# shravan-d/SculptMate

Measured on AMD Instinct MI355X. Metric: meshes/sec + ms/image, TripoSR 256^3 grid, at 1/2/4/8 MI355X, higher is better.
Workload: dtype fp32-equivalent (bf16 3-limb split, 24 bits, fp32 accumulate) density MLP / f32 tables, SiLU, marching cubes / bf16 transformer [filtered grid: an fp16 one-product pass decides the SIGN away from the level, every value marching cubes reads carries the three-limb value: mesh bit-identical to the full

## Files before the change

include/sculpt_hip.h:

```cpp
#ifndef SCULPT_HIP_H
#define SCULPT_HIP_H

#include <stddef.h>
#include <stdint.h>

#ifdef __cplusplus
extern "C" {
#endif

#define SCULPT_ABI_VERSION 4

typedef void *sculpt_stream_t;

int sculpt_version(void);
const char *sculpt_source_digest(void);
const char *sculpt_last_error(void);
int sculpt_device_count(void);
int sculpt_stream_create_cu_mask(int first_cu, int n_cus, sculpt_stream_t *stream_out);
int sculpt_stream_destroy(sculpt_stream_t stream);

size_t sculpt_mlp_packed_bytes(int in_channels, int n_hidden_64);
int sculpt_mlp_pack(const float *const *W_host, const float *const *b_host, int n_layers,
                    const int *dims_host, void *packed_host, size_t packed_bytes);

int sculpt_triplane_query(const float *planes, int C, int H, int W, const void *mlp_packed,
                          int n_hidden_64, const float *points, int64_t N, float radius, float density_bias,
                          float *density, float *features, float *density_act, float *color,
                          sculpt_stream_t stream);

#define SCULPT_QUERY_ALIGN_CORNERS 1u
#define SCULPT_QUERY_CHANNEL_LAST 2u
int sculpt_planes_channel_last(const float *planes , int C, int H, int W, float *out ,
                               sculpt_stream_t stream);
int sculpt_triplane_query_ex(const float *planes, int C, int H, int W, const void *mlp_packed,
                             int n_hidden_64, const float *points, int64_t N, float radius, float density_bias,
                             unsigned flags, float *density, float *features, float *density_act, float *color,
                             sculpt_stream_t stream);

int sculpt_render_rays(const float *planes_cl , int C, int H, int W,
                       const void *mlp_packed, int n_hidden_64,
                       const float *rays_o, const float *rays_d , int64_t n_rays,
                       float radius, float density_bias,
                       const float *t_vals , int S,
                       float *comp_rgb ,
                       float *opacity ,
                       float *z_vals  ,
                       float *weights ,
                       sculpt_stream_t stream);

int sculpt_render_passes(const float *planes_cl , int C, int H, int W,
                         const void *mlp_packed, int n_hidden_64,
                         const float *rays_o, const float *rays_d , int64_t n_rays,
                         float radius, float density_bias,
                         const float *t_vals , int S,
                         float *comp_rgb ,
                         float *opacity ,
                         float *z_vals  ,
                         float *weights ,
                         float *depth_sum  ,
                         float *normal_sum ,
                         float *premul     ,
                         sculpt_stream_t stream);

int sculpt_bake_scene_color(const float *planes_cl , int C, int H, int W,
                            const void *mlp_packed, int n_hidden_64,
                            const float *v_pos , size_t nv,
                            const void *faces , int faces_i64, size_t nf,
                            const float *rast , int res,
                            float radius,
                            float *color , uint8_t *mask ,
                            sculpt_stream_t stream);

int sculpt_corner_tangents(const float *v_pos , size_t nv, const void *faces , int faces_i64, size_t nf,
                           const float *uvs , const float *corner_normals ,
                           float *tangents , sculpt_stream_t stream);

int sculpt_bake_scene_normal(const float *planes_cl , int C, int H, int W,
                             const void *mlp_packed, int n_hidden_64,
                             const float *v_pos , size_t nv,
                             const void *faces , int faces_i64, size_t nf,
                             const float *rast , int res,
                             float radius,
                             const float *corner_normals , const float *corner_tangents ,
                             float *normal , uint8_t *mask ,
                             sculpt_stream_t stream);

int sculpt_triplane_density_grad(const float *planes_cl , int C, int H, int W,
                                 const void *mlp_packed, int n_hidden_64,
                                 const float *points , long long N, float radius, int flags ,
                                 float *grad , float *normal , float *density ,
                                 sculpt_stream_t stream);

size_t sculpt_density_grid_workspace_bytes(int R, int nx);
int sculpt_plane_features(const float *planes, int C, int H, int W, const void *mlp_packed,
                          const float *axis_coords, int R, int x_begin, int x_end, float radius,
                          void *workspace, sculpt_stream_t stream);
int sculpt_plane_features_ex(const float *planes, int C, int H, int W, const void *mlp_packed,
                             const float *axis_coords, int R, int x_begin, int x_end, float radius, unsigned flags,
                             void *workspace, sculpt_stream_t stream);
int sculpt_density_grid(const void *mlp_packed, int n_hidden_64, int R, int x_begin, int x_end,
                        float density_bias, float out_add, const void *workspace, float *out,
                        sculpt_stream_t stream);
#define SCULPT_DENSITY_BF16L3 4u
int sculpt_density_grid_ex(const void *mlp_packed, int n_hidden_64, int R, int x_begin, int x_end,
                           float density_bias, float out_add, const void *workspace, float *out, unsigned flags,
                           sculpt_stream_t stream);
#define SCULPT_FILTER_STATS_WORDS 12
#define SCULPT_FILTER_COARSE_FP16 8u
#define SCULPT_FILTER_MARK_ALL 16u
#define SCULPT_FILTER_PASS_A 32u
#define SCULPT_FILTER_PASS_B 64u
#define SCULPT_FILTER_PASS_C 128u
size_t sculpt_density_filter_workspace_bytes(int R, int nx);
int sculpt_density_grid_filtered(const void *mlp_packed, int n_hidden_64, int R, int x_begin, int x_end, float density_bias,
                                 float out_add, float margin, const void *workspace, void *filter_workspace, float *out,
                                 unsigned flags, sculpt_stream_t stream);
size_t sculpt_density_filter_sign_offset(int R, int nx);
int sculpt_density_filter_stats(const void *filter_workspace, int32_t *stats , sculpt_stream_t stream);
int sculpt_grid_decode(const void *mlp_packed, int n_hidden_64, int R, int x_begin, int x_end, float density_bias,
                       float out_add, const void *workspace, float *density_act, float *features, sculpt_stream_t stream);

#define SCULPT_MC_FACES_I64 1u
#define SCULPT_MC_REFERENCE_ORDER 2u
#define SCULPT_MC_USE_CLASSIC 4u
#define SCULPT_MC_SLAB 8u
#define SCULPT_MC_SLAB_HALO_LOW 16u
#define SCULPT_MC_SIGNED 32u
#define SCULPT_ERR_MC_LEVEL 11
#define SCULPT_ERR_MC_EMPTY 12
#define SCULPT_ERR_MC_NAN 13
#define SCULPT_ERR_MC_WORKSPACE 14
#define SCULPT_ERR_MC_NO_COUNT 15

size_t sculpt_mc_workspace_bytes(int n0, int n1, int n2);
size_t sculpt_mc_workspace_bytes_for(int n0, int n1, int n2, int64_t max_active_cells);
int sculpt_mc_count(const float *vol, int n0, int n1, int n2, double level, unsigned flags,
                    void *workspace, int64_t *n_verts_host, int64_t *n_faces_host,
                    float *minmax_host , sculpt_stream_t stream);
int sculpt_mc_emit(const float *vol, int n0, int n1, int n2, double level, unsigned flags,
                   void *workspace, float vert_div, float vert_mul, float vert_add,
                   int axis0_offset ,
                   float *verts, void *faces, int *top_plane_map , sculpt_stream_t stream);
int sculpt_mc_count_launch(const float *vol, int n0, int n1, int n2, double level, unsigned flags, void *workspace,
                           sculpt_stream_t stream);
int sculpt_mc_count_launch_signed(const float *vol, const uint32_t *sign_planes, int words_per_row, int n0, int n1, int n2,
                                  double level, unsigned flags, void *workspace, sculpt_stream_t stream);
int sculpt_mc_count_read(int n0, int n1, int n2, double level, unsigned flags, const void *workspace, int64_t *n_verts_host,
                         int64_t *n_faces_host, float *minmax_host , sculpt_stream_t stream);
int sculpt_mc_count_launch_for(const float *vol, const uint32_t *sign_planes , int words_per_row, int n0, int n1, int n2,
                               double level, unsigned flags, int64_t max_active_cells, void *workspace, sculpt_stream_t stream);
int sculpt_mc_count_read_ex(int n0, int n1, int n2, double level, unsigned flags, const void *workspace, int64_t *n_verts_host,
                            int64_t *n_faces_host, float *minmax_host , int64_t *n_active_host ,
                            sculpt_stream_t stream);
int sculpt_mc_emit_capped(const float *vol, int n0, int n1, int n2, double level, unsigned flags, void *workspace, float vert_div,
                          float vert_mul, float vert_add, int axis0_offset, float *verts, int64_t cap_verts, void *faces,
                          int64_t cap_faces, int *top_plane_map , sculpt_stream_t stream);

#define SCULPT_SN_INDEX_I64 1u
#define SCULPT_ERR_SN_EMPTY 17
size_t sculpt_surface_nets_workspace_bytes(int n0, int n1, int n2);
int sculpt_surface_nets_count(const float *vol, const uint32_t *sign_planes , int words_per_row, int n0, int n1, int n2,
                              double level, unsigned flags, void *workspace, int64_t *n_verts_host, int64_t *n_quads_host,
                              sculpt_stream_t stream);
int sculpt_surface_nets_emit(const float *vol, int n0, int n1, int n2, double level, unsigned flags, void *workspace, float vert_div,
                             float vert_mul, float vert_add, float *verts, void *quads , void *faces ,
                             sculpt_stream_t stream);

#define SCULPT_CC_KEEP_NONE 0
#define SCULPT_CC_KEEP_LARGEST 1
#define SCULPT_CC_KEEP_MIN_FACES 2
#define SCULPT_CC_KEEP_FRACTION 3
#define SCULPT_ERR_MESH_COMPONENTS 16
size_t sculpt_mesh_components_workspace_bytes(int64_t n_vertices, int64_t n_faces);
int sculpt_mesh_components_launch(const void *faces, int faces_i64, int64_t n_faces, int64_t n_vertices, int rule, int64_t min_faces,
                                  double fraction, void *workspace, sculpt_stream_t stream);
int sculpt_mesh_components_read(const void *workspace, int64_t *counts_host );
int sculpt_mesh_components_compact(const float *vertices, const void *faces, int faces_i64, int64_t n_faces, int64_t n_vertices,
                                   void *workspace, float *out_vertices, int64_t cap_vertices, void *out_faces, int64_t cap_faces,
                                   int64_t *vertex_index, int64_t *face_index, sculpt_stream_t stream);
// ... 387 lines not shown
```

sculptmate_amd/_lib.py:

```python
import ctypes
import os

import torch

_HERE = os.path.dirname(os.path.abspath(__file__))
SO_PATH = os.path.join(_HERE, "libsculpt_hip.so")


class SculptError(RuntimeError):
    def __init__(self, msg, code=1):
        super().__init__(msg)
        self.code = code


if not os.path.exists(SO_PATH):
    raise ImportError(
        "sculptmate_amd: %s is missing -- build it with `python -m sculptmate_amd.build` "
        "(or __graft_entry__.build()); there is no CPU fallback." % SO_PATH)


def _load_matching_library():
    from . import build as _build

    if os.environ.get("SCULPT_ALLOW_STALE_LIB") == "1":
# ... 202 lines not shown
    "sculpt_catmull_classify": (_i, [_vp, _vp, _vp, _vp, _vp]),
    "sculpt_catmull_refine": (_i, [_vp, _vp, _vp, _vp, _vp, _i, _vp, _vp, _vp, _vp, _vp]),
    "sculpt_surface_closest": (_i, [_vp, _i64, _vp, _vp, _vp, _i64, _vp, _vp, _vp, _vp, _d, _vp, _vp, _vp, _vp]),
    "sculpt_surface_cells": (_i, [_vp, _i64, _vp, _vp, _vp]),
    "sculpt_surface_pack": (_i, [_vp, _vp, _i64, _vp, _vp]),
    "sculpt_surface_weights": (_i, [_vp, _vp, _i64, _vp, _vp, _vp, _vp]),
    "sculpt_surface_sample": (_i, [_vp, _vp, _i64, _vp, _i64, ctypes.c_uint64, _vp, _vp, _vp, _vp]),
    "sculpt_surface_winding": (_i, [_vp, _i64, _vp, _vp, _vp, _i64, _vp, _vp, _vp, _vp, _vp, _vp]),
    "sculpt_surface_winding_lattice": (_i, [_vp, _d, _i, _i, _i, _vp, _vp, _i64, _vp, _vp, _vp, _vp, _vp, _vp, _vp]),
    "sculpt_lattice_active_blocks": (_i64, [_i, _i, _i]),
    "sculpt_lattice_active_corners": (_i, [_vp, _i, _i, _i, _vp, _vp, _i64, _vp]),
    "sculpt_sdf_fill": (_i, [_vp, _vp, _i, _i, _i, _vp, _vp, _i64, _d, _vp]),
    "sculpt_surface_ray_cast": (_i, [_vp, _vp, _i64, _vp, _vp, _vp, _i64, _vp, _vp, _vp, _vp, _d, _d, _d, _vp, _vp, _vp, _vp]),
    "sculpt_surface_occlusion": (_i, [_vp, _vp, _i64, _vp, _vp, _i, _f, _f, _vp, _vp, _i64, _vp, _vp, _vp, _vp, _d, _vp, _vp]),
    "sculpt_bake_occlusion": (_i, [_vp, _i, _vp, _sz, _vp, _i, _sz, _vp, _vp, _i, _f, _f, _f, _vp, _vp, _i64, _vp, _vp, _vp, _vp, _d, _vp,
                                   _vp, _vp]),
    "sculpt_surface_render": (_i, [_vp, _vp, _i64, _i64, _i64, _vp, _vp, _i64, _vp, _vp, _vp, _vp, _d, _vp, _f, _vp, _d, _vp, _vp]),
    "sculpt_triplane_project": (_i, [_vp, _i, _i, _i, _vp, _i, _vp, ctypes.c_longlong, _f, _i, _f, _i, _f, _f, _vp, _vp, _vp, _vp, _vp]),
    "sculpt_mesh_unfold": (_i, [_vp, _vp, _vp, _i64, _i64, _i, _vp, _vp, _vp]),
    "sculpt_bake_scene_surface": (_i, [_vp, _i, _i, _i, _vp, _i, _vp, _sz, _vp, _i, _sz, _vp, _i, _f, _vp, _vp, _f, _i, _f, _f, _vp, _vp,
                                       _vp, _vp, _vp, _vp, _vp]),
    "sculpt_bake_texel_list_workspace_bytes": (_sz, [_i]),
    "sculpt_bake_texel_list": (_i, [_vp, _sz, _vp, _i, _sz, _vp, _vp, _i, _vp, _vp, _vp, _vp, _vp, _vp, _vp, _vp, _vp, _vp, _vp]),
    "sculpt_triplane_project_along": (_i, [_vp, _i, _i, _i, _vp, _i, _vp, _vp, ctypes.c_longlong, _vp, _f, _i, _f, _i, _f, _f, _vp,
                                           ctypes.c_longlong, _vp, _vp, _vp, _vp, _vp]),
    "rasterize_cpu": (None, [_vp, _sz, _vp, _sz, ctypes.c_longlong, _vp]),
    "interpolate_cpu": (None, [_vp, _sz, _vp, _sz, _vp, ctypes.c_longlong, _vp]),
}

for _name, (_res, _args) in SIGNATURES.items():
    _fn = getattr(lib, _name)
    _fn.restype = _res
    _fn.argtypes = _args

def rmd_undo_bytes(nv):
    return ((nv + 3) & ~3) + 4


class RmdTopo(ctypes.Structure):
    _fields_ = [("F", _vp), ("skeys", _vp), ("she", _vp), ("es", _vp), ("fe", _vp), ("vfs", _vp), ("vfc", _vp), ("bnd", _vp),
                ("nf", _i64), ("nv", _i64), ("ne", _i64)]


class CatmullTopo(ctypes.Structure):
    _fields_ = [("F", _vp), ("skeys", _vp), ("she", _vp), ("es", _vp), ("fe", _vp), ("vfs", _vp), ("vfc", _vp),
                ("nf", _i64), ("nv", _i64), ("ne", _i64), ("k", ctypes.c_int32)]


class RenderMaterial(ctypes.Structure):
    _fields_ = [("uvs", _vp), ("texture", _vp), ("normal_map", _vp), ("corner_normals", _vp), ("corner_tangents", _vp),
                ("occlusion_map", _vp), ("vertex_colors", _vp), ("vertex_normals", _vp), ("vertex_occlusion", _vp),
                ("texture_res", _i), ("normal_map_res", _i), ("occlusion_map_res", _i), ("vertex_color_channels", _i)]


class RenderOutputs(ctypes.Structure):
    _fields_ = [("color", _vp), ("shaded", _vp), ("opacity", _vp), ("rgba", _vp), ("depth", _vp), ("normal", _vp), ("occlusion", _vp),
                ("face", _vp)]


class LnFold(ctypes.Structure):
    _fields_ = [("stats_in", _vp), ("slots_in", _i), ("colsum", _vp), ("eps", _f), ("stats_out", _vp), ("stats_ld", _i),
                ("rows_per_image", _i)]


MC_FACES_I64 = 1
MC_REFERENCE_ORDER = 2
MC_USE_CLASSIC = 4
MC_SLAB = 8
MC_SLAB_HALO_LOW = 16
MC_SIGNED = 32
LIMBS_BF16X3, LIMBS_F16X2 = 0, 1
ERR_MC_LEVEL = 11
ERR_MC_EMPTY = 12
ERR_MC_NAN = 13
ERR_MC_WORKSPACE = 14
ERR_MC_NO_COUNT = 15
ERR_MESH_COMPONENTS = 16
SN_INDEX_I64 = 1
ERR_SN_EMPTY = 17
CC_KEEP_NONE, CC_KEEP_LARGEST, CC_KEEP_MIN_FACES, CC_KEEP_FRACTION = 0, 1, 2, 3
EPI_NONE, EPI_GELU, EPI_GEGLU, EPI_RELU = 0, 1, 2, 3
QUERY_ALIGN_CORNERS = 1
QUERY_CHANNEL_LAST = 2
DENSITY_BF16L3 = 4
FILTER_COARSE_FP16 = 8
FILTER_MARK_ALL = 16
FILTER_PASS_A, FILTER_PASS_B, FILTER_PASS_C = 32, 64, 128
F32_EXACT, F32_BF16L3 = 0, 1


def last_error():
    return (lib.sculpt_last_error() or b"").decode("utf-8", "replace")


def check(rc):
    if rc != 0:
        raise SculptError(last_error() or ("sculpt error %d" % rc), rc)


def form_has(var, token):
    return any(t == token or t.startswith(token + "=") for t in os.environ.get(var, "").split(",") if t)
```

sculptmate_amd/csrc/triplane.hip:

```cpp
#include <math.h>
#include <stdlib.h>
#include <string.h>

#include <vector>

#include "common.h"
#include "triplane_mlp.h"

namespace sculpt {

static inline uint16_t host_f32_to_bf16(float f) {
    uint32_t u;
    memcpy(&u, &f, 4);
    if ((u & 0x7fffffffu) > 0x7f800000u) return (uint16_t)((u >> 16) | 0x40);
    return (uint16_t)((u + 0x7fffu + ((u >> 16) & 1u)) >> 16);
}
static inline float host_bf16_to_f32(uint16_t v) {
    uint32_t u = (uint32_t)v << 16;
    float f;
    memcpy(&f, &u, 4);
    return f;
}

static void pack_layout(int K0, int NH, MlpPackHeader *hd) {
// ... 85 lines not shown
            if (features) { features[3 * n] = f0; features[3 * n + 1] = f1; features[3 * n + 2] = f2; }
            if (color) {
                color[3 * n] = color_f(f0);
                color[3 * n + 1] = color_f(f1);
                color[3 * n + 2] = color_f(f2);
            }
        }
    }
}

template <int C, bool AC = false>
__global__ __launch_bounds__(256) void plane_features_kernel(
    const float *__restrict__ planes, int H, int W, const float *__restrict__ blob,
    const float *__restrict__ axis, int R, int x_begin, int nx, float radius, float span,
    float *__restrict__ FA, float *__restrict__ FB, float *__restrict__ FC) {
    __shared__ __attribute__((aligned(16))) float wl[C][64];
    __shared__ __attribute__((aligned(16))) float bl[64];
    const MlpPackHeader hd = *reinterpret_cast<const MlpPackHeader *>(blob);
    const int K0 = hd.K0;
    const int lane = threadIdx.x & 63, w = threadIdx.x >> 6;
    const int bgroups = (R + 3) / 4;
    const long perA = (long)((nx + 63) / 64) * bgroups, perC = (long)((R + 63) / 64) * bgroups;
    int k, na;
    long rest;
    float *dst;
    {
        const long blk = blockIdx.x;
        if (blk < perA) { k = 0; rest = blk; na = nx; dst = FA; }
        else if (blk < 2 * perA) { k = 1; rest = blk - perA; na = nx; dst = FB; }
        else { k = 2; rest = blk - 2 * perA; na = R; dst = FC; }
    }
    (void)perC;
    const int a = (int)(rest / bgroups) * 64 + lane;
    const int b = (int)(rest % bgroups) * 4 + w;
    for (int i = threadIdx.x; i < C * 64; i += 256) {
        const int c = i >> 6, jj = i & 63;
        const int hh = jj >> 5, tt = (jj >> 4) & 1, rr = jj & 15;
        wl[c][jj] = blob[hd.off_w0raw + (long)nrow(tt, rr, hh) * K0 + k * C + c];
    }
    if (threadIdx.x < 64) {
        const int jj = threadIdx.x, hh = jj >> 5, tt = (jj >> 4) & 1, rr = jj & 15;
        bl[jj] = (k == 0) ? blob[hd.off_b0raw + nrow(tt, rr, hh)] : 0.f;
    }
    __syncthreads();
    if (b >= R) return;
    const bool live = a < na;
    const int ac = live ? a : na - 1;
    const int ia = (k == 2) ? ac : ac + x_begin;
    const float gx = to_unit(axis[ia], radius, span), gy = to_unit(axis[b], radius, span);
    Tap1 tx = tap_of<AC>(gx, W), ty = tap_of<AC>(gy, H);
    const float wx = tx.w1, ex = 1.0f - wx, wy = ty.w1, ey = 1.0f - wy;
    const int x0 = tx.i0, x1 = x0 + 1, y0 = ty.i0, y1 = y0 + 1;
    const bool vx0 = x0 >= 0 && x0 < W, vx1 = x1 >= 0 && x1 < W;
    const bool vy0 = y0 >= 0 && y0 < H, vy1 = y1 >= 0 && y1 < H;
    const int cx0 = min(max(x0, 0), W - 1), cx1 = min(max(x1, 0), W - 1);
    const int cy0 = min(max(y0, 0), H - 1), cy1 = min(max(y1, 0), H - 1);
    const float wnw = (vy0 && vx0) ? ey * ex : 0.f, wne = (vy0 && vx1) ? ey * wx : 0.f;
    const float wsw = (vy1 && vx0) ? wy * ex : 0.f, wse = (vy1 && vx1) ? wy * wx : 0.f;
    const int o00 = cy0 * W + cx0, o01 = cy0 * W + cx1, o10 = cy1 * W + cx0, o11 = cy1 * W + cx1;
    float s[64];
#pragma unroll
    for (int jj = 0; jj < 64; ++jj) s[jj] = bl[jj];
    const float *P = planes + (long)k * C * H * W;
#pragma unroll 2
    for (int c = 0; c < C; ++c, P += (long)H * W) {
        float v = P[o00] * wnw;
        v += P[o01] * wne;
        v += P[o10] * wsw;
        v += P[o11] * wse;
        const f32x4 *wr = reinterpret_cast<const f32x4 *>(&wl[c][0]);
#pragma unroll
        for (int q = 0; q < 16; ++q) {
            const f32x4 ww = wr[q];
            s[4 * q] = fmaf(ww[0], v, s[4 * q]);
            s[4 * q + 1] = fmaf(ww[1], v, s[4 * q + 1]);
            s[4 * q + 2] = fmaf(ww[2], v, s[4 * q + 2]);
            s[4 * q + 3] = fmaf(ww[3], v, s[4 * q + 3]);
        }
    }
    if (live) {
        f32x4 *o = reinterpret_cast<f32x4 *>(dst + ((long)a * R + b) * 64);
#pragma unroll
        for (int q = 0; q < 16; ++q) o[q] = f32x4{s[4 * q], s[4 * q + 1], s[4 * q + 2], s[4 * q + 3]};
    }
}


template <int NT>
__global__ __launch_bounds__(NT) void density_grid_kernel(
    const float *__restrict__ blob, const float *__restrict__ FA, const float *__restrict__ FB,
    const float *__restrict__ FC, int R, int nx, float density_bias, float out_add, float *__restrict__ out,
    int xcd_band) {
    extern __shared__ __attribute__((aligned(16))) float smem[];
    const MlpPackHeader hd = *reinterpret_cast<const MlpPackHeader *>(blob);
    const int NH = hd.NH;
    load_weights_to_lds(smem, blob, hd);
    const LdsView L = lds_view(smem, NH);

    const int lane = threadIdx.x & 63, nwave = blockDim.x >> 6;
    const int wave = __builtin_amdgcn_readfirstlane(threadIdx.x >> 6);
    const int p = lane & 31, h = lane >> 5;
    const int nzb = (R + 31) / 32;
    const long ntiles = (long)nx * nzb * R;
    const long nw_total = (long)gridDim.x * nwave;
    long wid = (long)blockIdx.x * nwave + wave;
    if (xcd_band && gridDim.x % 8 == 0)
        wid = ((long)(blockIdx.x & 7) * (gridDim.x >> 3) + (blockIdx.x >> 3)) * nwave + wave;
    const long t_begin = ntiles * wid / nw_total, t_end = ntiles * (wid + 1) / nw_total;
    int iy = (int)(t_begin % R);
    int zb = (int)((t_begin / R) % nzb), ixl = (int)((t_begin / R) / nzb);

    for (long t = t_begin; t < t_end; ++t, ++iy) {
        if (iy == R) {
            iy = 0;
            if (++zb == nzb) { zb = 0; ++ixl; }
        }
        const int iz = zb * 32 + p;
        const int izc = min(iz, R - 1);
        f32x16 x0, x1, y0, y1;
        load_row32(FA + ((long)ixl * R + iy) * 64 + h * 32, x0, x1);
        load_row32(FB + ((long)ixl * R + izc) * 64 + h * 32, y0, y1);
        x0 += y0; x1 += y1;
        load_row32(FC + ((long)iy * R + izc) * 64 + h * 32, y0, y1);
        x0 += y0; x1 += y1;
        x0 = silu16(x0); x1 = silu16(x1);
        hidden_layers(L, NH, lane, h, x0, x1);
        const float d = last_dot(L, 0, h, x0, x1);
        if (h == 0 && iz < R) out[((long)ixl * R + iy) * R + iz] = exp_f(d + density_bias) + out_add;
    }
}

__global__ __launch_bounds__(1024) void lattice_decode_kernel(
    const float *__restrict__ blob, const float *__restrict__ FA, const float *__restrict__ FB,
    const float *__restrict__ FC, int R, int nx, float density_bias, float out_add, float *__restrict__ out,
    float *__restrict__ features) {
    extern __shared__ __attribute__((aligned(16))) float smem[];
    const MlpPackHeader hd = *reinterpret_cast<const MlpPackHeader *>(blob);
    const int NH = hd.NH;
    load_weights_to_lds(smem, blob, hd);
    const LdsView L = lds_view(smem, NH);
    const int lane = threadIdx.x & 63, nwave = blockDim.x >> 6;
    const int wave = __builtin_amdgcn_readfirstlane(threadIdx.x >> 6);
    const int p = lane & 31, h = lane >> 5;
    const long plane = (long)R * R;
    const long tpx = (plane + 31) / 32, ntiles = (long)nx * tpx;
    const long nw_total = (long)gridDim.x * nwave;
    long wid = (long)blockIdx.x * nwave + wave;
    if (gridDim.x % 8 == 0) wid = ((long)(blockIdx.x & 7) * (gridDim.x >> 3) + (blockIdx.x >> 3)) * nwave + wave;
    const long t_begin = ntiles * wid / nw_total, t_end = ntiles * (wid + 1) / nw_total;
    for (long t = t_begin; t < t_end; ++t) {
        const int ixl = (int)(t / tpx);
        const long flat = (t - (long)ixl * tpx) * 32 + p;
        const long fc = min(flat, plane - 1);
        const int iy = (int)(fc / R), iz = (int)(fc - (long)iy * R);
        f32x16 x0, x1, y0, y1;
        load_row32(FA + ((long)ixl * R + iy) * 64 + h * 32, x0, x1);
        load_row32(FB + ((long)ixl * R + iz) * 64 + h * 32, y0, y1);
        x0 += y0; x1 += y1;
        load_row32(FC + fc * 64 + h * 32, y0, y1);
        x0 += y0; x1 += y1;
        x0 = silu16(x0); x1 = silu16(x1);
        hidden_layers(L, NH, lane, h, x0, x1);
        const float d = last_dot(L, 0, h, x0, x1);
        const float f0 = last_dot(L, 1, h, x0, x1), f1 = last_dot(L, 2, h, x0, x1), f2 = last_dot(L, 3, h, x0, x1);
        if (h == 0 && flat < plane) {
            const long idx = (long)ixl * plane + flat;
// ... 235 lines not shown
        for (int T = 0; T < 2; ++T)
            for (int s4 = 0; s4 < 4; ++s4)
                for (int lane = 0; lane < 64; ++lane)
                    for (int j = 0; j < 8; ++j) {
                        const int k = 16 * s4 + 8 * (j >> 2) + 4 * (lane >> 5) + (j & 3);
                        const float w = Wl[(size_t)(32 * T + (lane & 31)) * HID + k];
                        const float w1 = host_bf16_to_f32(host_f32_to_bf16(w));
                        const float r1 = w - w1;
                        const float w2 = host_bf16_to_f32(host_f32_to_bf16(r1));
                        w3[(size_t)l * 4096 + (((T * 4 + s4) * 64 + lane) * 8) + j] = host_f32_to_bf16(r1 - w2);
                    }
    }
    _Float16 *x3h = reinterpret_cast<_Float16 *>(o + hd.off_x3h);
    for (int l = 0; l < NH; ++l) {
        const float *Wl = Wh[l + 1];
        for (int part = 0; part < 2; ++part)
            for (int T = 0; T < 2; ++T)
                for (int s4 = 0; s4 < 4; ++s4)
                    for (int lane = 0; lane < 64; ++lane)
                        for (int j = 0; j < 8; ++j) {
                            const int k = 16 * s4 + 8 * (j >> 2) + 4 * (lane >> 5) + (j & 3);
                            const float w = Wl[(size_t)(32 * T + (lane & 31)) * HID + k];
                            const _Float16 hi = (_Float16)w;
                            const _Float16 lo = (_Float16)(w - (float)hi);
                            x3h[(size_t)l * 8192 + ((((part * 2 + T) * 4 + s4) * 64 + lane) * 8) + j] = part ? lo : hi;
                        }
    }
    return 0;
}

static size_t lds_bytes_for(int NH) { return (size_t)(NH * 4096 + (NH + 1) * 64 + 256 + 4) * sizeof(float); }

int sculpt_triplane_query(const float *planes, int C, int H, int W, const void *mlp_packed,
                          int n_hidden_64, const float *points, int64_t N, float radius, float density_bias,
                          float *density, float *features, float *density_act, float *color,
                          sculpt_stream_t stream) {
    return sculpt_triplane_query_ex(planes, C, H, W, mlp_packed, n_hidden_64, points, N, radius, density_bias, 0u,
                                    density, features, density_act, color, stream);
}

int sculpt_triplane_query_ex(const float *planes, int C, int H, int W, const void *mlp_packed,
                             int n_hidden_64, const float *points, int64_t N, float radius, float density_bias,
                             unsigned flags, float *density, float *features, float *density_act, float *color,
                             sculpt_stream_t stream) {
    hipStream_t st = as_stream(stream);
    SC_REQUIRE(C == 40, "triplane_query: built for C=40 channels per plane (got %d)", C);
    SC_REQUIRE(planes && mlp_packed, "triplane_query: null input");
    if (N <= 0) return 0;
    SC_REQUIRE(points, "triplane_query: null points");
    SC_REQUIRE(n_hidden_64 >= 0, "triplane_query: bad n_hidden_64");
    size_t lds = lds_bytes_for(n_hidden_64);
    SC_REQUIRE(lds <= 160 * 1024, "triplane_query: %d hidden layers do not fit LDS", n_hidden_64);
    const bool ac = flags & SCULPT_QUERY_ALIGN_CORNERS, cl = flags & SCULPT_QUERY_CHANNEL_LAST;
    const size_t a0_bytes = (size_t)3 * C * 64 * sizeof(float);
    const int a0_lds = (cl && lds + a0_bytes <= 160 * 1024) ? 1 : 0;
    if (a0_lds) lds += a0_bytes;
    auto kern = cl ? (ac ? query_points_kernel<40, true, true> : query_points_kernel<40, false, true>)
                   : (ac ? query_points_kernel<40, true, false> : query_points_kernel<40, false, false>);
    SC_HIP(hipFuncSetAttribute(reinterpret_cast<const void *>(kern), hipFuncAttributeMaxDynamicSharedMemorySize, (int)lds));
    const long ntiles = (N + 31) / 32;
    const int grid = (int)std::min<long>((ntiles + 7) / 8, num_cus());
    const float span = (float)((double)radius - (double)(-radius));
    hipLaunchKernelGGL(kern, dim3(grid), dim3(512), lds, st, planes, H, W,
                       reinterpret_cast<const float *>(mlp_packed), points, (long)N, radius, span,
                       density_bias, density, features, density_act, color, a0_lds);
    SC_LAUNCH_CHECK();
    return 0;
}

size_t sculpt_density_grid_workspace_bytes(int R, int nx) {
    return ((size_t)2 * nx * R + (size_t)R * R) * 64 * sizeof(float);
}

int sculpt_plane_features(const float *planes, int C, int H, int W, const void *mlp_packed,
                          const float *axis_coords, int R, int x_begin, int x_end, float radius,
                          void *workspace, sculpt_stream_t stream) {
    return sculpt_plane_features_ex(planes, C, H, W, mlp_packed, axis_coords, R, x_begin, x_end, radius, 0u, workspace, stream);
}

int sculpt_plane_features_ex(const float *planes, int C, int H, int W, const void *mlp_packed,
                             const float *axis_coords, int R, int x_begin, int x_end, float radius, unsigned flags,
                             void *workspace, sculpt_stream_t stream) {
    hipStream_t st = as_stream(stream);
    SC_REQUIRE((flags & ~SCULPT_QUERY_ALIGN_CORNERS) == 0, "plane_features: planes are channel-first [3][C][H][W]; unknown flags %u", flags);
    SC_REQUIRE(C == 40, "plane_features: built for C=40 channels per plane (got %d)", C);
    SC_REQUIRE(planes && mlp_packed && axis_coords && workspace, "plane_features: null argument");
    SC_REQUIRE(R >= 2 && x_begin >= 0 && x_end <= R && x_begin < x_end, "plane_features: bad range [%d,%d) of %d", x_begin, x_end, R);
    const int nx = x_end - x_begin;
    float *FA = reinterpret_cast<float *>(workspace);
    float *FB = FA + (size_t)nx * R * 64;
    float *FC = FB + (size_t)nx * R * 64;
    const float span = (float)((double)radius - (double)(-radius));
    const long pairs = 2L * nx * R + (long)R * R;
    (void)pairs;
    const long pf_bg = (R + 3) / 4;
    const long pf_blocks = 2 * (long)((nx + 63) / 64) * pf_bg + (long)((R + 63) / 64) * pf_bg;
    if (flags & SCULPT_QUERY_ALIGN_CORNERS)
        hipLaunchKernelGGL((plane_features_kernel<40, true>), dim3((unsigned)pf_blocks), dim3(256), 0, st, planes, H, W,
                           reinterpret_cast<const float *>(mlp_packed), axis_coords, R, x_begin, nx, radius,
                           span, FA, FB, FC);
    else
        hipLaunchKernelGGL((plane_features_kernel<40, false>), dim3((unsigned)pf_blocks), dim3(256), 0, st, planes, H, W,
                           reinterpret_cast<const float *>(mlp_packed), axis_coords, R, x_begin, nx, radius,
                           span, FA, FB, FC);
    SC_LAUNCH_CHECK();
    return 0;
}

int sculpt_density_grid(const void *mlp_packed, int n_hidden_64, int R, int x_begin, int x_end,
                        float density_bias, float out_add, const void *workspace, float *out,
                        sculpt_stream_t stream) {
    return sculpt_density_grid_ex(mlp_packed, n_hidden_64, R, x_begin, x_end, density_bias, out_add, workspace, out, 0u,
                                  stream);
}

int sculpt_density_grid_ex(const void *mlp_packed, int n_hidden_64, int R, int x_begin, int x_end,
                           float density_bias, float out_add, const void *workspace, float *out, unsigned flags,
                           sculpt_stream_t stream) {
    hipStream_t st = as_stream(stream);
    SC_REQUIRE(mlp_packed && workspace && out, "density_grid: null argument");
    SC_REQUIRE((flags & ~SCULPT_DENSITY_BF16L3) == 0, "density_grid: unknown flags %u (the two-limb modes 1 / 2 were removed)", flags);
    SC_REQUIRE(R >= 2 && x_begin >= 0 && x_end <= R && x_begin < x_end, "density_grid: bad range [%d,%d) of %d", x_begin, x_end, R);
    SC_REQUIRE(n_hidden_64 >= 0, "density_grid: bad n_hidden_64");
    const size_t lds = lds_bytes_for(n_hidden_64);
    SC_REQUIRE(lds <= 160 * 1024, "density_grid: %d hidden layers do not fit LDS", n_hidden_64);
    const int nx = x_end - x_begin;
    const float *FA = reinterpret_cast<const float *>(workspace);
    const float *FB = FA + (size_t)nx * R * 64;
    const float *FC = FB + (size_t)nx * R * 64;
    const long ntiles = (long)nx * ((R + 31) / 32) * R;
    if ((flags & SCULPT_DENSITY_BF16L3) && n_hidden_64 >= 1) {
        const bool kstep = !form_has("SCULPT_DENSITY_FORM", "nokstep");
        constexpr int nt = 1024;
        auto kern = kstep ? density_grid_l3k_kernel<1024> : density_grid_l3_kernel<1024>;
        SC_HIP(hipFuncSetAttribute(reinterpret_cast<const void *>(kern), hipFuncAttributeMaxDynamicSharedMemorySize, (int)lds));
        const int nwave = nt / 64;
        const int grid = (int)std::min<long>((ntiles + nwave - 1) / nwave, num_cus());
        hipLaunchKernelGGL(kern, dim3(grid), dim3(nt), lds, st, reinterpret_cast<const float *>(mlp_packed), FA, FB, FC, R, nx,
                           density_bias, out_add, out);
        SC_LAUNCH_CHECK();
        return 0;
    }
    {
        SC_HIP(hipFuncSetAttribute(reinterpret_cast<const void *>(density_grid_kernel<1024>), hipFuncAttributeMaxDynamicSharedMemorySize, (int)lds));
        const int grid = (int)std::min<long>((ntiles + 15) / 16, num_cus());
        hipLaunchKernelGGL(density_grid_kernel<1024>, dim3(grid), dim3(1024), lds, st,
                           reinterpret_cast<const float *>(mlp_packed), FA, FB, FC, R, nx, density_bias, out_add, out, 1);
    }
    SC_LAUNCH_CHECK();
    return 0;
}

int sculpt_grid_decode(const void *mlp_packed, int n_hidden_64, int R, int x_begin, int x_end, float density_bias,
                       float out_add, const void *workspace, float *density_act, float *features, sculpt_stream_t stream) {
    hipStream_t st = as_stream(stream);
    SC_REQUIRE(mlp_packed && workspace && (density_act || features), "grid_decode: null argument");
    SC_REQUIRE(R >= 2 && x_begin >= 0 && x_end <= R && x_begin < x_end, "grid_decode: bad range [%d,%d) of %d", x_begin, x_end, R);
    SC_REQUIRE(n_hidden_64 >= 0, "grid_decode: bad n_hidden_64");
    const size_t lds = lds_bytes_for(n_hidden_64);
    SC_REQUIRE(lds <= 160 * 1024, "grid_decode: %d hidden layers do not fit LDS", n_hidden_64);
    const int nx = x_end - x_begin;
    const float *FA = reinterpret_cast<const float *>(workspace);
    const float *FB = FA + (size_t)nx * R * 64;
    const float *FC = FB + (size_t)nx * R * 64;
    const long ntiles = (long)nx * (((long)R * R + 31) / 32);
    SC_HIP(hipFuncSetAttribute(reinterpret_cast<const void *>(lattice_decode_kernel), hipFuncAttributeMaxDynamicSharedMemorySize, (int)lds));
    const int grid = (int)std::min<long>((ntiles + 15) / 16, num_cus());
    hipLaunchKernelGGL(lattice_decode_kernel, dim3(grid), dim3(1024), lds, st, reinterpret_cast<const float *>(mlp_packed), FA, FB, FC,
                       R, nx, density_bias, out_add, density_act, features);
    SC_LAUNCH_CHECK();
    return 0;
}

}
```

Measured before the change: 125.9.

## Add row-oriented plane features kernel with LDS transpose for coalesced stores

Adds a new default plane-features kernel. Each lane samples all 40 channels once into registers, then computes output features in groups of 4 from weights read straight from global memory, and stages them through per-wave LDS. The staging transposes the results so that stores to the [a][b][64] workspace are coalesced 16-byte writes rather than one lane writing a whole 64-float row. The old kernel stays available behind a new REFERENCE flag. In exchange, the loop over 64 outputs is serialised and weights are loaded per group from memory instead of from LDS.

```diff
diff --git a/include/sculpt_hip.h b/include/sculpt_hip.h
--- a/include/sculpt_hip.h
+++ b/include/sculpt_hip.h
@@ -95,6 +95,7 @@
 int sculpt_plane_features(const float *planes, int C, int H, int W, const void *mlp_packed,
                           const float *axis_coords, int R, int x_begin, int x_end, float radius,
                           void *workspace, sculpt_stream_t stream);
+#define SCULPT_PLANE_FEATURES_REFERENCE 4u
 int sculpt_plane_features_ex(const float *planes, int C, int H, int W, const void *mlp_packed,
                              const float *axis_coords, int R, int x_begin, int x_end, float radius, unsigned flags,
                              void *workspace, sculpt_stream_t stream);
diff --git a/sculptmate_amd/_lib.py b/sculptmate_amd/_lib.py
--- a/sculptmate_amd/_lib.py
+++ b/sculptmate_amd/_lib.py
@@ -308,6 +308,7 @@
 EPI_NONE, EPI_GELU, EPI_GEGLU, EPI_RELU = 0, 1, 2, 3
 QUERY_ALIGN_CORNERS = 1
 QUERY_CHANNEL_LAST = 2
+PLANE_FEATURES_REFERENCE = 4
 DENSITY_BF16L3 = 4
 FILTER_COARSE_FP16 = 8
 FILTER_MARK_ALL = 16
diff --git a/sculptmate_amd/csrc/triplane.hip b/sculptmate_amd/csrc/triplane.hip
--- a/sculptmate_amd/csrc/triplane.hip
+++ b/sculptmate_amd/csrc/triplane.hip
@@ -191,6 +191,94 @@
         f32x4 *o = reinterpret_cast<f32x4 *>(dst + ((long)a * R + b) * 64);
 #pragma unroll
         for (int q = 0; q < 16; ++q) o[q] = f32x4{s[4 * q], s[4 * q + 1], s[4 * q + 2], s[4 * q + 3]};
+    }
+}
+
+template <int C, bool AC = false>
+__global__ __launch_bounds__(256) void plane_features_rows_kernel(
+    const float *__restrict__ planes, int H, int W, const float *__restrict__ blob,
+    const float *__restrict__ axis, int R, int x_begin, int nx, float radius, float span,
+    float *__restrict__ FA, float *__restrict__ FB, float *__restrict__ FC) {
+    constexpr int NJ = 32, LD = NJ + 4;
+    __shared__ __attribute__((aligned(16))) float xch[4][64][LD];
+    const MlpPackHeader hd = *reinterpret_cast<const MlpPackHeader *>(blob);
+    const int K0 = hd.K0;
+    const int lane = threadIdx.x & 63, w = threadIdx.x >> 6;
+    const int bgroups = (R + 3) / 4;
+    const long perA = (long)((nx + 63) / 64) * bgroups;
+    int k, na;
+    long rest;
+    float *dst;
+    {
+        const long blk = blockIdx.x;
+        if (blk < perA) { k = 0; rest = blk; na = nx; dst = FA; }
+        else if (blk < 2 * perA) { k = 1; rest = blk - perA; na = nx; dst = FB; }
+        else { k = 2; rest = blk - 2 * perA; na = R; dst = FC; }
+    }
+    const int a0 = (int)(rest / bgroups) * 64, a = a0 + lane;
+    const int b = (int)(rest % bgroups) * 4 + w;
+    if (b >= R) return;
+    const int ac = a < na ? a : na - 1;
+    const int ia = (k == 2) ? ac : ac + x_begin;
+    const float gx = to_unit(axis[ia], radius, span), gy = to_unit(axis[b], radius, span);
+    Tap1 tx = tap_of<AC>(gx, W), ty = tap_of<AC>(gy, H);
+    const float wx = tx.w1, ex = 1.0f - wx, wy = ty.w1, ey = 1.0f - wy;
+    const int x0 = tx.i0, x1 = x0 + 1, y0 = ty.i0, y1 = y0 + 1;
+    const bool vx0 = x0 >= 0 && x0 < W, vx1 = x1 >= 0 && x1 < W;
+    const bool vy0 = y0 >= 0 && y0 < H, vy1 = y1 >= 0 && y1 < H;
+    const int cx0 = min(max(x0, 0), W - 1), cx1 = min(max(x1, 0), W - 1);
+    const int cy0 = min(max(y0, 0), H - 1), cy1 = min(max(y1, 0), H - 1);
+    const float wnw = (vy0 && vx0) ? ey * ex : 0.f, wne = (vy0 && vx1) ? ey * wx : 0.f;
+    const float wsw = (vy1 && vx0) ? wy * ex : 0.f, wse = (vy1 && vx1) ? wy * wx : 0.f;
+    const int o00 = cy0 * W + cx0, o01 = cy0 * W + cx1, o10 = cy1 * W + cx0, o11 = cy1 * W + cx1;
+    float v[C];
+    {
+        const float *P = planes + (long)k * C * H * W;
+#pragma unroll
+        for (int c = 0; c < C; ++c, P += (long)H * W) {
+            float t = P[o00] * wnw;
+            t += P[o01] * wne;
+            t += P[o10] * wsw;
+            t += P[o11] * wse;
+            v[c] = t;
+        }
+    }
+    const float *wk = blob + hd.off_w0raw + k * C;
+    const float *bk = blob + hd.off_b0raw;
+    float(*X)[LD] = xch[w];
+    for (int half = 0; half < 64 / NJ; ++half) {
+#pragma unroll 1
+        for (int g = 0; g < NJ / 4; ++g) {
+            const float *wr[4];
+            float s[4];
+#pragma unroll
+            for (int q = 0; q < 4; ++q) {
+                const int jj = half * NJ + 4 * g + q;
+                const int n = nrow((jj >> 4) & 1, jj & 15, jj >> 5);
+                wr[q] = wk + (long)n * K0;
+                s[q] = (k == 0) ? bk[n] : 0.f;
+            }
+#pragma unroll
+            for (int c = 0; c < C; ++c) {
+#pragma unroll
+                for (int q = 0; q < 4; ++q) s[q] = fmaf(wr[q][c], v[c], s[q]);
+            }
+            *reinterpret_cast<f32x4 *>(&X[lane][4 * g]) = f32x4{s[0], s[1], s[2], s[3]};
+        }
+        __builtin_amdgcn_fence(__ATOMIC_RELEASE, "wavefront");
+        __builtin_amdgcn_wave_barrier();
+        __builtin_amdgcn_fence(__ATOMIC_ACQUIRE, "wavefront");
+        constexpr int LPR = NJ / 4, RPI = 64 / LPR;
+        const int piece = lane % LPR;
+#pragma unroll
+        for (int i = 0; i < 64 / RPI; ++i) {
+            const int r = i * RPI + lane / LPR;
+            const f32x4 val = *reinterpret_cast<const f32x4 *>(&X[r][4 * piece]);
+            if (a0 + r < na) *reinterpret_cast<f32x4 *>(dst + ((long)(a0 + r) * R + b) * 64 + half * NJ + 4 * piece) = val;
+        }
+        __builtin_amdgcn_fence(__ATOMIC_RELEASE, "wavefront");
+        __builtin_amdgcn_wave_barrier();
+        __builtin_amdgcn_fence(__ATOMIC_ACQUIRE, "wavefront");
     }
 }
 
@@ -592,7 +680,8 @@
                              const float *axis_coords, int R, int x_begin, int x_end, float radius, unsigned flags,
                              void *workspace, sculpt_stream_t stream) {
     hipStream_t st = as_stream(stream);
-    SC_REQUIRE((flags & ~SCULPT_QUERY_ALIGN_CORNERS) == 0, "plane_features: planes are channel-first [3][C][H][W]; unknown flags %u", flags);
+    SC_REQUIRE((flags & ~(SCULPT_QUERY_ALIGN_CORNERS | SCULPT_PLANE_FEATURES_REFERENCE)) == 0,
+               "plane_features: planes are channel-first [3][C][H][W]; unknown flags %u", flags);
     SC_REQUIRE(C == 40, "plane_features: built for C=40 channels per plane (got %d)", C);
     SC_REQUIRE(planes && mlp_packed && axis_coords && workspace, "plane_features: null argument");
     SC_REQUIRE(R >= 2 && x_begin >= 0 && x_end <= R && x_begin < x_end, "plane_features: bad range [%d,%d) of %d", x_begin, x_end, R);
@@ -605,14 +694,12 @@
     (void)pairs;
     const long pf_bg = (R + 3) / 4;
     const long pf_blocks = 2 * (long)((nx + 63) / 64) * pf_bg + (long)((R + 63) / 64) * pf_bg;
-    if (flags & SCULPT_QUERY_ALIGN_CORNERS)
-        hipLaunchKernelGGL((plane_features_kernel<40, true>), dim3((unsigned)pf_blocks), dim3(256), 0, st, planes, H, W,
-                           reinterpret_cast<const float *>(mlp_packed), axis_coords, R, x_begin, nx, radius,
-                           span, FA, FB, FC);
-    else
-        hipLaunchKernelGGL((plane_features_kernel<40, false>), dim3((unsigned)pf_blocks), dim3(256), 0, st, planes, H, W,
-                           reinterpret_cast<const float *>(mlp_packed), axis_coords, R, x_begin, nx, radius,
-                           span, FA, FB, FC);
+    const bool ac = flags & SCULPT_QUERY_ALIGN_CORNERS;
+    auto kern = (flags & SCULPT_PLANE_FEATURES_REFERENCE)
+                    ? (ac ? plane_features_kernel<40, true> : plane_features_kernel<40, false>)
+                    : (ac ? plane_features_rows_kernel<40, true> : plane_features_rows_kernel<40, false>);
+    hipLaunchKernelGGL(kern, dim3((unsigned)pf_blocks), dim3(256), 0, st, planes, H, W,
+                       reinterpret_cast<const float *>(mlp_packed), axis_coords, R, x_begin, nx, radius, span, FA, FB, FC);
     SC_LAUNCH_CHECK();
     return 0;
 }
```

Measured after the change: 126.5 (median of 6 runs). Within noise of the previous version (+0.5%).
